# lashhw/rtcuda

Hardware: NVIDIA B200
Metric: Mrays/s (extend+shadow) (higher is better)
Workload: dtype f32

## Files before the change

rtcuda_b200/csrc/rtb_cuda.cu:

```cuda
#include <cuda_runtime.h>
#include <dlfcn.h>
#include <nccl.h>

#include <cctype>
#include <cstdlib>
#include <mutex>

#include <cub/block/block_scan.cuh>
#include <cub/device/device_radix_sort.cuh>
#include <cub/device/device_scan.cuh>
#include <cub/device/device_select.cuh>

#include "rtb_engine.h"

#define RTB_CUDA_CHECK(expr)                                                                              \
    do {                                                                                                  \
        cudaError_t e_ = (expr);                                                                          \
        if (e_ != cudaSuccess)                                                                            \
            throw rtb::Error(e_ == cudaErrorMemoryAllocation ? RTB_ERR_OOM : RTB_ERR_CUDA,                \
                             std::string(#expr) + ": " + cudaGetErrorName(e_) + " (" + cudaGetErrorString(e_) + ")"); \
    } while (0)

namespace rtb {

constexpr int kBlock = 256;
#ifndef RTB_TRACE_BLOCK
#define RTB_TRACE_BLOCK 128
#endif
constexpr int kTraceBlock = RTB_TRACE_BLOCK;
#ifndef RTB_TRACE_MIN_BLOCKS
#define RTB_TRACE_MIN_BLOCKS (1024 / RTB_TRACE_BLOCK)
#endif
constexpr int kTraceBlocksPerSm = RTB_TRACE_MIN_BLOCKS;

template <class F>
__global__ void __launch_bounds__(kBlock) k_for(int n, F f) {
    const int i = blockIdx.x * kBlock + threadIdx.x;
    if (i < n) f(i);
}

__global__ void __launch_bounds__(kBlock) k_generate(WaveState W, RenderConsts rc) {
    const int n = generate_count(W);
    for (int i = blockIdx.x * kBlock + threadIdx.x; i < n; i += gridDim.x * kBlock) generate_body(W, rc, i);
}

__device__ __forceinline__ void prefetch_l2(const void *p) { asm volatile("prefetch.global.L2 [%0];" ::"l"(p)); }

__device__ __forceinline__ void cp_async16(void *smem, const void *gmem) {
    asm volatile("cp.async.cg.shared.global [%0], [%1], 16;" ::"r"((unsigned)__cvta_generic_to_shared(smem)), "l"(gmem));
}
#ifndef RTB_SHADE_BLOCK
#define RTB_SHADE_BLOCK 128
#endif
constexpr int kShadeBlock = RTB_SHADE_BLOCK;
#ifndef RTB_SHADE_MATTE_BLOCKS
#define RTB_SHADE_MATTE_BLOCKS 2
#endif
constexpr int shade_blocks_per_sm(int type) { return ((type == RTB_MIRROR || type == RTB_GLASS) ? 3 : RTB_SHADE_MATTE_BLOCKS) * (256 / kShadeBlock); }
template <int TYPE, bool EXT = false>
__global__ void __launch_bounds__(kShadeBlock, shade_blocks_per_sm(TYPE)) k_shade(WaveState W, SceneView S, RenderConsts rc, bool shadows) {
    __shared__ float4 stage[2][3][kShadeBlock];
    const int n = W.c->n_mat[TYPE];
    const int stride = gridDim.x * kShadeBlock, t = threadIdx.x;
    ShadeTally tally; tally.extend = 0u; tally.shadow = 0u;
    int i = blockIdx.x * kShadeBlock + t;
    if (i < n) {
        const size_t q = (size_t)W.qbase[TYPE] + (size_t)i;
        cp_async16(&stage[0][0][t], W.ma + q); cp_async16(&stage[0][1][t], W.mb + q); cp_async16(&stage[0][2][t], W.mc + q);
    }
    asm volatile("cp.async.commit_group;");
    for (int buf = 0; i < n; i += stride, buf ^= 1) {
        if (i + stride < n) {
            const size_t q = (size_t)W.qbase[TYPE] + (size_t)(i + stride);
            cp_async16(&stage[buf ^ 1][0][t], W.ma + q); cp_async16(&stage[buf ^ 1][1][t], W.mb + q); cp_async16(&stage[buf ^ 1][2][t], W.mc + q);
        }
        asm volatile("cp.async.commit_group;");
        asm volatile("cp.async.wait_group 1;" ::: "memory");
        const float4 a4 = stage[buf][0][t], b4 = stage[buf][1][t], h4 = stage[buf][2][t];
        F4 a, b, hr;
        a.x = a4.x; a.y = a4.y; a.z = a4.z; a.w = a4.w; b.x = b4.x; b.y = b4.y; b.z = b4.z; b.w = b4.w;
        hr.x = h4.x; hr.y = h4.y; hr.z = h4.z; hr.w = h4.w;
        shade_item<TYPE, EXT>(W, S, rc, shadows, i, a, b, hr, tally);
    }
    asm volatile("cp.async.wait_all;" ::: "memory");
    tally_flush(W.c, tally);
}

__global__ void k_control(WaveState W, bool shadows) { control_body(W, shadows); }

struct FetchTuning {
    int refill;
    int chunk;
    int prefetch;
    int tri_step;
};

struct alignas(16) WarpScratch {
    float4 ro[32];
    float4 rd[32];
    float4 fin[32];
    float4 res[32];
    uint2 item[32];
};
template <bool ANY>
__device__ __forceinline__ void pooled_triangles(WarpScratch &ws, const Bvh8View &B, Traversal<ANY, false> &T, uint32_t tx,
                                                 uint32_t ty, bool &has, bool &pending, const unsigned lane,
                                                 const unsigned lanes_below) {
    while (__any_sync(0xffffffffu, ty != 0u)) {
        const int cnt = min(__popc(ty), 3);
        const unsigned b0 = __ballot_sync(0xffffffffu, cnt & 1), b1 = __ballot_sync(0xffffffffu, cnt & 2);
        const int first = __popc(b0 & lanes_below) + 2 * __popc(b1 & lanes_below);
        const int total = __popc(b0) + 2 * __popc(b1);
        const int take = max(0, min(cnt, 32 - first));
#pragma unroll
        for (int k = 0; k < 3; ++k) {
            if (k < take) {
                const int bit = 31 - __clz(ty);
                ty &= ~(1u << bit);
                ws.item[first + k] = make_uint2(tx + (uint32_t)bit, lane);
            }
        }
        __syncwarp();
        if ((int)lane < min(total, 32)) {
            const uint2 it = ws.item[lane];
            const float4 o = ws.ro[it.y], d = ws.rd[it.y];
            const Tri48 tr = load_tri(B.tris, (int)it.x);
            float u, v;
            const float t = tri_candidate(tr, v3(o.x, o.y, o.z), v3(d.x, d.y, d.z), u, v);
            ws.res[lane] = make_float4(t, u, v, __int_as_float((int)it.x));
        }
        __syncwarp();
#pragma unroll
        for (int k = 0; k < 3; ++k) {
            if (k < take && has) {
                const float4 c = ws.res[first + k];
                if (T.accept(B, __float_as_int(c.w), c.x, c.y, c.z)) {
                    ty = 0u; has = false; pending = true;
                }
            }
        }
        __syncwarp();
    }
}
template <bool ANY>
__device__ __forceinline__ void own_triangles(const Bvh8View &B, Traversal<ANY, false> &T, uint32_t tx, uint32_t ty, bool &has,
                                              bool &pending) {
    while (ty) {
        const int bit = 31 - __clz(ty);
        ty &= ~(1u << bit);
        const int idx = (int)(tx + (uint32_t)bit);
        const Tri48 tr = load_tri(B.tris, idx);
        float u, v;
        const float t = tri_candidate(tr, T.r.o, T.r.d, u, v);
        if (T.accept(B, idx, t, u, v)) { has = false; pending = true; break; }
    }
}

struct LocalStackK : LocalStack {
    __device__ explicit LocalStackK(uint2 *) {}
};
template <int N>
struct HybridStack {
    uint2 *s;
    uint32_t x[kStackSize - N], y[kStackSize - N];
    __device__ explicit HybridStack(uint2 *column) : s(column) {}
    __device__ __forceinline__ void put(int i, uint32_t a, uint32_t b) {
        if (i < N) s[i * kTraceBlock] = make_uint2(a, b);
        else { x[i - N] = a; y[i - N] = b; }
    }
    __device__ __forceinline__ void get(int i, uint32_t &a, uint32_t &b) const {
        if (i < N) { const uint2 v = s[i * kTraceBlock]; a = v.x; b = v.y; }
        else { a = x[i - N]; b = y[i - N]; }
    }
};
template <bool ANY, bool POOL, bool INST = false, class STACK = LocalStackK>
__device__ __forceinline__ void persistent_trace(WarpScratch &ws, const WaveState &W, const SceneView &S, FetchTuning tune, uint2 *ws_stack = nullptr) {
    const int n = ANY ? W.c->n_shadow : W.c->n_extend;
    int32_t *head = ANY ? &W.c->shadow_head : &W.c->extend_head;
    const unsigned lane = threadIdx.x & 31u;
    const unsigned lanes_below = (1u << lane) - 1u;
    Traversal<ANY, false, INST> T;
    STACK st(ws_stack);
    bool has = false, exhausted = false, pending = false;
    int qi = 0;
    int chunk_next = 0, chunk_end = 0;
    uint32_t tx = 0u, ty = 0u;
    while (true) {
        if (pending) {
            asm volatile("cp.async.wait_all;" ::: "memory");
            const float4 fw = ws.fin[lane];
            if (ANY) {
                if (!T.found) {
                    const V3 L = v3(fw.x, fw.y, fw.z);
                    if (finite3(L)) accum_add(W, __float_as_uint(fw.w), L);
                }
            } else if (T.hit.tri < 0) {
                if (W.has_env) extend_miss(W, __float_as_uint(ws.ro[lane].w), v3(fw.x, fw.y, fw.z));
            } else {
                const int mat = INST ? hit_material(S, T.hit.tri, T.hit_inst) : S.tri_meta[T.hit.tri].material;
                const int type = mat >> 24;
                const int j = hit_queue_push(W, type);
                if (INST) W.hit_inst[j] = T.hit_inst;
                F4 beta; beta.x = fw.x; beta.y = fw.y; beta.z = fw.z; beta.w = fw.w;
                const float4 o = ws.ro[lane], d = ws.rd[lane];
                F4 ma; ma.x = d.x; ma.y = d.y; ma.z = d.z; ma.w = o.w;
                F4 mb; mb.x = beta.x; mb.y = beta.y; mb.z = beta.z; mb.w = d.w;
                F4 mc; mc.x = i2f(mat); mc.y = T.hit.u; mc.z = T.hit.v; mc.w = i2f(T.hit.tri);
                W.ma[j] = ma; W.mb[j] = mb; W.mc[j] = mc;
                if (W.mis) { W.mis[2 * (size_t)j] = beta.w; W.mis[2 * (size_t)j + 1] = T.hit.t; }
            }
            pending = false;
        }
        unsigned need = __ballot_sync(0xffffffffu, !has);
        for (int round = 0; round < 2 && need != 0u && !exhausted; ++round) {
            if (chunk_next >= chunk_end) {
                int base = 0;
                if (lane == 0u) base = atomicAdd(head, tune.chunk);
                base = __shfl_sync(0xffffffffu, base, 0);
                chunk_next = base;
                chunk_end = min(base + tune.chunk, n);
                if (base >= n) { exhausted = true; break; }
                if (tune.prefetch) {
                    for (int i = base + (int)lane; i < chunk_end; i += 32) {
                        if (ANY) { prefetch_l2(W.sh_o + i); prefetch_l2(W.sh_d + i); }
                        else { prefetch_l2(W.ea + i); prefetch_l2(W.eb + i); prefetch_l2(W.ec + i); }
                    }
                }
            }
            const int idx = chunk_next + __popc(need & lanes_below);
            if (!has && idx < chunk_end) {
                if (ANY) {
                    const F4 o = ldg(W.sh_o + idx), d = ldg(W.sh_d + idx);
                    if (o.w > 0.f) {
                        cp_async16(&ws.fin[lane], W.sh_L + idx);
                        ws.ro[lane] = make_float4(o.x, o.y, o.z, 0.f);
                        ws.rd[lane] = make_float4(d.x, d.y, d.z, 0.f);
                        T.init(xyz(o), xyz(d), o.w, f2i(d.w));
                        qi = idx; has = true; ty = 0u;
                    }
                } else {
                    const F4 a = ldg(W.ea + idx), b = ldg(W.eb + idx);
                    if (f2u(a.w) != kHolePixel) {
                        cp_async16(&ws.fin[lane], W.ec + idx);
                        ws.ro[lane] = make_float4(a.x, a.y, a.z, a.w);
                        ws.rd[lane] = make_float4(b.x, b.y, b.z, b.w);
                        T.init(xyz(a), xyz(b), FLT_MAX, -1);
                        qi = idx; has = true; ty = 0u;
                    }
                }
            }
            chunk_next = min(chunk_next + __popc(need), chunk_end);
            need = __ballot_sync(0xffffffffu, !has);
        }
        unsigned act = __ballot_sync(0xffffffffu, has);
        if (act == 0u) {
            if (exhausted) return;
            continue;
        }
        const int keep_going = exhausted ? 1 : tune.refill;
        do {
            if constexpr (INST) {
                if (has && ty == 0u) T.node_part(S.bvh, st, tx, ty);
                if (has && T.cur < 0) {
                    if (ty != 0u) {
                        const float4 o = ws.ro[lane], d = ws.rd[lane];
                        T.enter_instance(S.bvh, st, tx, ty, v3(o.x, o.y, o.z), v3(d.x, d.y, d.z));
                    }
                } else if (ty != 0u) {
// ... 11 lines not shown
                    else if (two && T.accept(S.bvh, idx2, t2, u2, v2)) { has = false; pending = true; ty = 0u; }
                }
                if (has && ty == 0u) {
                    const float4 o = ws.ro[lane], d = ws.rd[lane];
                    if (!T.advance_inst(st, tx, ty, v3(o.x, o.y, o.z), v3(d.x, d.y, d.z))) { has = false; pending = true; }
                }
            } else if constexpr (POOL) {
                tx = 0u; ty = 0u;
                if (has) T.node_part(S.bvh, st, tx, ty);
                pooled_triangles<ANY>(ws, S.bvh, T, tx, ty, has, pending, lane, lanes_below);
                ty = 0u;
                if (has && !T.advance(st)) { has = false; pending = true; }
            } else if (tune.tri_step > 0) {
                if (has && ty == 0u) T.node_part(S.bvh, st, tx, ty);
                if (tune.tri_step == 2) {
                  if (ty != 0u) {
                    const int bit1 = 31 - __clz(ty);
                    ty &= ~(1u << bit1);
                    const bool two = ty != 0u;
                    const int bit2 = two ? 31 - __clz(ty) : bit1;
                    ty &= ~(1u << bit2);
                    const int idx1 = (int)(tx + (uint32_t)bit1), idx2 = (int)(tx + (uint32_t)bit2);
                    const Tri48 tr1 = load_tri(S.bvh.tris, idx1), tr2 = load_tri(S.bvh.tris, idx2);
                    float u1, v1, u2, v2;
                    const float t1 = tri_candidate(tr1, T.r.o, T.r.d, u1, v1);
                    const float t2 = tri_candidate(tr2, T.r.o, T.r.d, u2, v2);
                    if (T.accept(S.bvh, idx1, t1, u1, v1)) { has = false; pending = true; ty = 0u; }
                    else if (two && T.accept(S.bvh, idx2, t2, u2, v2)) { has = false; pending = true; ty = 0u; }
                  }
                } else {
#pragma unroll 1
                for (int k = 0; k < tune.tri_step && ty != 0u; ++k) {
                    const int bit = 31 - __clz(ty);
                    ty &= ~(1u << bit);
                    const int idx = (int)(tx + (uint32_t)bit);
                    const Tri48 tr = load_tri(S.bvh.tris, idx);
                    float u, v;
                    const float t = tri_candidate(tr, T.r.o, T.r.d, u, v);
                    if (T.accept(S.bvh, idx, t, u, v)) { has = false; pending = true; ty = 0u; }
                }
                }
                if (has && ty == 0u && !T.advance(st)) { has = false; pending = true; }
            } else {
                tx = 0u; ty = 0u;
                if (has) T.node_part(S.bvh, st, tx, ty);
                own_triangles<ANY>(S.bvh, T, tx, ty, has, pending);
                ty = 0u;
                if (has && !T.advance(st)) { has = false; pending = true; }
            }
            act = __ballot_sync(0xffffffffu, has);
        } while (__popc(act) >= keep_going);
    }
}
template <int WHICH, bool POOL, bool INST = false>
__global__ void __launch_bounds__(kTraceBlock, kTraceBlocksPerSm) k_trace(WaveState W, SceneView S, FetchTuning tune) {
    __shared__ WarpScratch scratch[kTraceBlock / 32];
    WarpScratch &ws = scratch[threadIdx.x >> 5];
    if (WHICH & 1) persistent_trace<false, POOL, INST>(ws, W, S, tune);
    if (WHICH == 3) __syncwarp();
    if (WHICH & 2) persistent_trace<true, POOL, INST>(ws, W, S, tune);
}
constexpr int kSmemStack = 8;
__global__ void __launch_bounds__(kTraceBlock, kTraceBlocksPerSm) k_trace_smem_stack(WaveState W, SceneView S, FetchTuning tune) {
    __shared__ WarpScratch scratch[kTraceBlock / 32];
    __shared__ uint2 sstack[kSmemStack][kTraceBlock];
    WarpScratch &ws = scratch[threadIdx.x >> 5];
    persistent_trace<false, false, false, HybridStack<kSmemStack>>(ws, W, S, tune, &sstack[0][threadIdx.x]);
    __syncwarp();
    persistent_trace<true, false, false, HybridStack<kSmemStack>>(ws, W, S, tune, &sstack[0][threadIdx.x]);
}
template <int WHICH>
static void launch_trace_kernel(int grid, cudaStream_t st, bool pooled, bool smem_stack, const WaveState &W, const SceneView &S, const FetchTuning &tune) {
    if (WHICH == 3 && smem_stack && !S.bvh.inst && !pooled) { k_trace_smem_stack<<<grid, kTraceBlock, 0, st>>>(W, S, tune); return; }
    if (S.bvh.inst) {
        k_trace<WHICH, false, true><<<grid, kTraceBlock, 0, st>>>(W, S, tune);
    } else if (pooled) k_trace<WHICH, true><<<grid, kTraceBlock, 0, st>>>(W, S, tune);
    else k_trace<WHICH, false><<<grid, kTraceBlock, 0, st>>>(W, S, tune);
}
template <bool COUNT>
__global__ void __launch_bounds__(kBlock) k_extend_flat(WaveState W, SceneView S) {
    const int i = blockIdx.x * kBlock + threadIdx.x;
    if (i < W.c->n_extend) extend_body<COUNT>(W, S, i);
}
template <bool COUNT>
__global__ void __launch_bounds__(kBlock) k_shadow_flat(WaveState W, SceneView S) {
    const int i = blockIdx.x * kBlock + threadIdx.x;
    if (i < W.c->n_shadow) shadow_body<COUNT>(W, S, i);
}

constexpr int kSetupBlock = 256;
__global__ void __launch_bounds__(kSetupBlock) k_prim_setup_tiled(PrimSetupArgs a) {
    __shared__ __align__(16) float vin[kSetupBlock * 9];
    __shared__ float4 rec[kSetupBlock * 3];
    const int b0 = blockIdx.x * kSetupBlock;
    const int cnt = min(kSetupBlock, a.n - b0);
    const float *src = a.vertices + 9 * (size_t)b0;
    if (cnt == kSetupBlock && (reinterpret_cast<uintptr_t>(src) & 15u) == 0) {
        const float4 *s4 = reinterpret_cast<const float4 *>(src);
        float4 *d4 = reinterpret_cast<float4 *>(vin);
        for (int t = threadIdx.x; t < kSetupBlock * 9 / 4; t += kSetupBlock) d4[t] = s4[t];
    } else {
        for (int t = threadIdx.x; t < cnt * 9; t += kSetupBlock) vin[t] = src[t];
    }
    __syncthreads();
    const int i = b0 + threadIdx.x;
    Tri48 tr;
    if (i < a.n) {
        const float *v = vin + 9 * threadIdx.x;
        tr = tri_from_vertices(v3(v[0], v[1], v[2]), v3(v[3], v[4], v[5]), v3(v[6], v[7], v[8]));
        float4 *r = rec + 3 * threadIdx.x;
        r[0] = make_float4(tr.p0x, tr.p0y, tr.p0z, tr.e1x);
        r[1] = make_float4(tr.e1y, tr.e1z, tr.e2x, tr.e2y);
        r[2] = make_float4(tr.e2z, tr.nx, tr.ny, tr.nz);
    }
    __syncthreads();
    float4 *dst = reinterpret_cast<float4 *>(a.tri_in + b0);
    for (int t = threadIdx.x; t < cnt * 3; t += kSetupBlock) dst[t] = rec[t];
    __shared__ int32_t part[kSetupBlock / 32][6];
    int32_t o[6] = {0x7fffffff, 0x7fffffff, 0x7fffffff, (int32_t)0x80000000, (int32_t)0x80000000, (int32_t)0x80000000};
    if (i < a.n) {
        V3 lo, hi;
        prim_setup_box(a, i, tr, lo, hi);
        o[0] = float_to_ordered(lo.x); o[1] = float_to_ordered(lo.y); o[2] = float_to_ordered(lo.z);
        o[3] = float_to_ordered(hi.x); o[4] = float_to_ordered(hi.y); o[5] = float_to_ordered(hi.z);
    }
#pragma unroll
    for (int k = 0; k < 3; ++k) { o[k] = __reduce_min_sync(0xffffffffu, o[k]); o[3 + k] = __reduce_max_sync(0xffffffffu, o[3 + k]); }
    if ((threadIdx.x & 31) == 0) for (int k = 0; k < 6; ++k) part[threadIdx.x >> 5][k] = o[k];
    __syncthreads();
    if (threadIdx.x < 6) {
// ... 350 lines not shown
    decltype(&ncclGetUniqueId) GetUniqueId = nullptr;
    decltype(&ncclCommInitRank) CommInitRank = nullptr;
    decltype(&ncclCommInitAll) CommInitAll = nullptr;
    decltype(&ncclCommDestroy) CommDestroy = nullptr;
    decltype(&ncclAllReduce) AllReduce = nullptr;
    decltype(&ncclReduce) Reduce = nullptr;
    decltype(&ncclGroupStart) GroupStart = nullptr;
    decltype(&ncclGroupEnd) GroupEnd = nullptr;
    decltype(&ncclGetErrorString) GetErrorString = nullptr;
    static Nccl &get() {
        static Nccl n;
        static std::once_flag once;
        std::call_once(once, [] {
            for (const char *name : {"libnccl.so.2", "libnccl.so"}) {
                n.lib = dlopen(name, RTLD_NOW | RTLD_GLOBAL);
                if (n.lib) break;
            }
            if (!n.lib) return;
#define RTB_NCCL_SYM(f) n.f = (decltype(n.f))dlsym(n.lib, "nccl" #f)
            RTB_NCCL_SYM(GetUniqueId); RTB_NCCL_SYM(CommInitRank); RTB_NCCL_SYM(CommInitAll); RTB_NCCL_SYM(CommDestroy);
            RTB_NCCL_SYM(AllReduce); RTB_NCCL_SYM(Reduce); RTB_NCCL_SYM(GroupStart); RTB_NCCL_SYM(GroupEnd); RTB_NCCL_SYM(GetErrorString);
#undef RTB_NCCL_SYM
        });
        if (!n.lib || !n.GetUniqueId || !n.CommInitRank || !n.CommInitAll || !n.CommDestroy || !n.AllReduce || !n.Reduce || !n.GroupStart ||
            !n.GroupEnd || !n.GetErrorString)
            throw Error(RTB_ERR_NO_DEVICE, "NCCL (libnccl.so.2) could not be loaded: multi-GPU entry points need it");
        return n;
    }
};
#define RTB_NCCL_CHECK(expr)                                                                                               \
    do {                                                                                                                   \
        ncclResult_t r_ = (expr);                                                                                          \
        if (r_ != ncclSuccess) throw rtb::Error(RTB_ERR_CUDA, std::string(#expr) + ": " + rtb::Nccl::get().GetErrorString(r_)); \
    } while (0)
static_assert(sizeof(ncclUniqueId) == RTB_COMM_ID_BYTES, "rtb.h: RTB_COMM_ID_BYTES must be sizeof(ncclUniqueId)");

struct NonNegative {
    __host__ __device__ bool operator()(const int32_t &v) const { return v >= 0; }
};

struct CudaBackend {
    int dev_ = -1;
    int num_sms_ = 0;
    cudaStream_t stream_ = nullptr;
    cudaStream_t streams_[kMaxPipelines] = {nullptr, nullptr};
    cudaEvent_t sync_ev_ = nullptr;
    cudaMemPool_t pool_mem_ = nullptr;
    int pipelines_ = 0;
    int blocks_trace_ = 0, blocks_generate_ = 0;
    int trace_blocks_per_sm_ = 1, trace_cap_ = 0, active_pipelines_ = 1;
    void *cub_temp_ = nullptr;
    size_t cub_temp_bytes_ = 0;
    int32_t *h_done_ = nullptr, *d_done_ = nullptr;
    FetchTuning tune_{24, 128, 1, 2};
    int pooled_ = 0;
    int fused_ = 1;
    int smem_stack_ = 0;
    WaveCache wave_cache_;
    WaveCache &wave_cache() { return wave_cache_; }
    int pool_ = 0;
    size_t pool_budget_ = 0;
    int ploc_tail_off_ = 0;
    int nn_tiled_off_ = 0;

    explicit CudaBackend(int device) {
        int count = 0;
        cudaError_t e = cudaGetDeviceCount(&count);
        if (e != cudaSuccess || count == 0)
            throw Error(RTB_ERR_NO_DEVICE, std::string("no CUDA device available (") + cudaGetErrorString(e) +
                                               "); rtcuda_b200 has no CPU fallback");
        if (device < 0 || device >= count) throw Error(RTB_ERR_INVALID, "device ordinal out of range");
        cudaDeviceProp prop;
        RTB_CUDA_CHECK(cudaGetDeviceProperties(&prop, device));
        if (prop.major != 10)
            throw Error(RTB_ERR_NO_DEVICE, std::string("device '") + prop.name + "' is sm_" + std::to_string(prop.major) +
                                               std::to_string(prop.minor) + "; this library is built for sm_100a (B200) only");
        dev_ = device;
        num_sms_ = prop.multiProcessorCount;
        RTB_CUDA_CHECK(cudaSetDevice(dev_));
        for (int k = 0; k < kMaxPipelines; ++k) RTB_CUDA_CHECK(cudaStreamCreateWithFlags(&streams_[k], cudaStreamDefault));
        stream_ = streams_[0];
        RTB_CUDA_CHECK(cudaEventCreateWithFlags(&sync_ev_, cudaEventDisableTiming));
        cudaMemPoolProps props = {};
        props.allocType = cudaMemAllocationTypePinned;
        props.handleTypes = cudaMemHandleTypeNone;
        props.location.type = cudaMemLocationTypeDevice;
        props.location.id = dev_;
        RTB_CUDA_CHECK(cudaMemPoolCreate(&pool_mem_, &props));
        unsigned long long keep = ~0ull;
        RTB_CUDA_CHECK(cudaMemPoolSetAttribute(pool_mem_, cudaMemPoolAttrReleaseThreshold, &keep));
        {
            size_t free_b = 0, total_b = 0;
            RTB_CUDA_CHECK(cudaMemGetInfo(&free_b, &total_b));
            pool_budget_ = free_b / 8;
        }
        RTB_CUDA_CHECK(cudaHostAlloc((void **)&h_done_, kMaxPipelines * sizeof(int32_t), cudaHostAllocMapped));
        RTB_CUDA_CHECK(cudaHostGetDevicePointer((void **)&d_done_, h_done_, 0));
        for (int k = 0; k < kMaxPipelines; ++k) h_done_[k] = 0;
        int per_sm = 0;
        RTB_CUDA_CHECK(cudaOccupancyMaxActiveBlocksPerMultiprocessor(&per_sm, k_trace<3, true>, kTraceBlock, 0));
        trace_blocks_per_sm_ = per_sm > 0 ? per_sm : 1;
        static const char *const names[] = {"refill", "chunk", "prefetch", "tri_step", "pooled", "fused", "smem_stack", "pipelines", "pool",
                                            "ploc_tail", "trace_blocks", "nn_tiled"};
        for (const char *nm : names) {
            std::string env = "RTB_";
            for (const char *c = nm; *c; ++c) env += (char)toupper((unsigned char)*c);
            if (const char *e = getenv(env.c_str())) set_option(nm, atoll(e));
        }
        blocks_trace_ = num_sms_ * trace_blocks_per_sm_;
        RTB_CUDA_CHECK(cudaOccupancyMaxActiveBlocksPerMultiprocessor(&per_sm, k_generate, kBlock, 0));
        blocks_generate_ = num_sms_ * (per_sm > 0 ? per_sm : 1);
    }
    ~CudaBackend() {
        if (dev_ < 0) return;
        cudaSetDevice(dev_);
        stream_ = streams_[0];
        for (int k = 0; k < kMaxPipelines; ++k) if (streams_[k]) cudaStreamSynchronize(streams_[k]);
        wave_cache_release(*this, wave_cache_);
        if (cub_temp_) cudaFreeAsync(cub_temp_, stream_);
        if (tail_counts_) cudaFreeAsync(tail_counts_, stream_);
        if (h_done_) cudaFreeHost(h_done_);
        if (sync_ev_) cudaEventDestroy(sync_ev_);
        for (int k = 0; k < kMaxPipelines; ++k) if (streams_[k]) { cudaStreamSynchronize(streams_[k]); cudaStreamDestroy(streams_[k]); }
        if (pool_mem_) cudaMemPoolDestroy(pool_mem_);
    }
    CudaBackend(const CudaBackend &) = delete;
    CudaBackend &operator=(const CudaBackend &) = delete;

    bool set_option(const std::string &name, long long v) {
        auto in = [&](long long lo, long long hi) { return v >= lo && v <= hi; };
        if (name == "refill") { if (!in(1, 32)) return false; tune_.refill = (int)v; }
        else if (name == "chunk") { if (!in(32, 1 << 20)) return false; tune_.chunk = (int)v; }
        else if (name == "prefetch") { if (!in(0, 1)) return false; tune_.prefetch = (int)v; }
        else if (name == "tri_step") { if (!in(0, 4)) return false; tune_.tri_step = (int)v; }
        else if (name == "pooled") { if (!in(-1, 1)) return false; pooled_ = (int)v; }
        else if (name == "fused") { if (!in(0, 1)) return false; fused_ = (int)v; }
        else if (name == "smem_stack") { if (!in(0, 1)) return false; smem_stack_ = (int)v; }
        else if (name == "pipelines") { if (!in(0, kMaxPipelines)) return false; pipelines_ = (int)v; }
        else if (name == "pool") { if (v != 0 && !in(1024, 1ll << 30)) return false; pool_ = (int)v; }
        else if (name == "ploc_tail") { if (!in(0, 1)) return false; ploc_tail_off_ = v == 0; }
        else if (name == "trace_blocks") { if (!in(0, trace_blocks_per_sm_)) return false; trace_cap_ = (int)v; }
        else if (name == "nn_tiled") { if (!in(0, 1)) return false; nn_tiled_off_ = v == 0; }
        else return false;
        return true;
    }
    bool get_option(const std::string &name, long long &v) const {
        if (name == "refill") v = tune_.refill;
        else if (name == "chunk") v = tune_.chunk;
        else if (name == "prefetch") v = tune_.prefetch;
        else if (name == "tri_step") v = tune_.tri_step;
        else if (name == "pooled") v = pooled_;
        else if (name == "fused") v = fused_;
        else if (name == "smem_stack") v = smem_stack_;
        else if (name == "pipelines") v = pipelines_;
        else if (name == "pool") v = pool_;
        else if (name == "ploc_tail") v = ploc_tail_off_ ? 0 : 1;
        else if (name == "trace_blocks") v = trace_cap_;
        else if (name == "nn_tiled") v = nn_tiled_off_ ? 0 : 1;
        else return false;
        return true;
    }
    int device() const { return dev_; }
    void make_current() { RTB_CUDA_CHECK(cudaSetDevice(dev_)); }
    void sync() { RTB_CUDA_CHECK(cudaStreamSynchronize(stream_)); }
    long long default_pool(size_t slot_bytes) const {
        if (pool_ > 0) return pool_;
        long long n = (long long)(pool_budget_ / (slot_bytes ? slot_bytes : 144));
        if (n < (1ll << 22)) n = 1ll << 22;
        if (n > (1ll << 28)) n = 1ll << 28;
        return n;
    }

    template <class T> T *alloc(size_t n) {
        void *p = nullptr;
        RTB_CUDA_CHECK(cudaMallocFromPoolAsync(&p, sizeof(T) * (n ? n : 1), pool_mem_, stream_));
        return (T *)p;
    }
    void free(void *p) { if (p) cudaFreeAsync(p, stream_); }
    template <class T> void upload(T *dst, const T *src, size_t n) {
        RTB_CUDA_CHECK(cudaMemcpyAsync(dst, src, sizeof(T) * n, cudaMemcpyHostToDevice, stream_));
        RTB_CUDA_CHECK(cudaStreamSynchronize(stream_));
    }
    template <class T> void download(T *dst, const T *src, size_t n) {
        RTB_CUDA_CHECK(cudaMemcpyAsync(dst, src, sizeof(T) * n, cudaMemcpyDeviceToHost, stream_));
        RTB_CUDA_CHECK(cudaStreamSynchronize(stream_));
    }
    template <class T> void copy(T *dst, const T *src, size_t n) {
        RTB_CUDA_CHECK(cudaMemcpyAsync(dst, src, sizeof(T) * n, cudaMemcpyDeviceToDevice, stream_));
    }
    template <class T> void zero(T *p, size_t n) { RTB_CUDA_CHECK(cudaMemsetAsync(p, 0, sizeof(T) * n, stream_)); }
    template <class T> void copy_from(CudaBackend &src_be, T *dst, const T *src, size_t n) {
        if (!n) return;
        if (src_be.dev_ == dev_) { copy(dst, src, n); return; }
        RTB_CUDA_CHECK(cudaMemcpyPeerAsync(dst, dev_, src, src_be.dev_, sizeof(T) * n, stream_));
    }
    struct Group { std::vector<ncclComm_t> comms; };
    static Group *group_create(const std::vector<CudaBackend *> &members) {
        Nccl &nc = Nccl::get();
        std::vector<int> devs;
        for (CudaBackend *b : members) devs.push_back(b->dev_);
        Group *g = new Group();
        g->comms.resize(members.size());
        ncclResult_t r = nc.CommInitAll(g->comms.data(), (int)devs.size(), devs.data());
        if (r != ncclSuccess) { delete g; throw Error(RTB_ERR_CUDA, std::string("ncclCommInitAll: ") + nc.GetErrorString(r)); }
        return g;
    }
    static void group_destroy(Group *g) {
        if (!g) return;
        for (ncclComm_t c : g->comms) if (c) Nccl::get().CommDestroy(c);
        delete g;
    }
    template <class T>
    static void group_reduce(Group *g, const std::vector<CudaBackend *> &members, const std::vector<T *> &bufs, size_t n, int root) {
        Nccl &nc = Nccl::get();
        const ncclDataType_t dt = sizeof(T) == 8 ? ncclInt64 : ncclFloat32;
        RTB_NCCL_CHECK(nc.GroupStart());
        for (size_t r = 0; r < members.size(); ++r) {
            ncclResult_t e = nc.Reduce(bufs[r], bufs[r], n, dt, ncclSum, root, g->comms[r], members[r]->streams_[0]);
            if (e != ncclSuccess) { nc.GroupEnd(); throw Error(RTB_ERR_CUDA, std::string("ncclReduce: ") + nc.GetErrorString(e)); }
        }
        RTB_NCCL_CHECK(nc.GroupEnd());
    }
    struct Comm { ncclComm_t comm = nullptr; int rank = 0, world = 1; };
    static void comm_unique_id(uint8_t *out) {
        ncclUniqueId id;
        RTB_NCCL_CHECK(Nccl::get().GetUniqueId(&id));
        memcpy(out, &id, sizeof id);
    }
    Comm *comm_create(const uint8_t *id_bytes, int rank, int world) {
        ncclUniqueId id;
        memcpy(&id, id_bytes, sizeof id);
        make_current();
        Comm *c = new Comm();
        c->rank = rank; c->world = world;
        ncclResult_t r = Nccl::get().CommInitRank(&c->comm, world, id, rank);
        if (r != ncclSuccess) { delete c; throw Error(RTB_ERR_CUDA, std::string("ncclCommInitRank: ") + Nccl::get().GetErrorString(r)); }
        return c;
    }
    static void comm_destroy(Comm *c) {
        if (!c) return;
        if (c->comm) Nccl::get().CommDestroy(c->comm);
        delete c;
    }
    template <class T> void comm_allreduce(Comm *c, T *buf, size_t n) {
        const ncclDataType_t dt = sizeof(T) == 8 ? ncclInt64 : ncclFloat32;
        RTB_NCCL_CHECK(Nccl::get().AllReduce(buf, buf, n, dt, ncclSum, c->comm, streams_[0]));
        RTB_CUDA_CHECK(cudaStreamSynchronize(streams_[0]));
    }

    template <class F> void launch(int n, F f) {
        if (n <= 0) return;
        k_for<F><<<(n + kBlock - 1) / kBlock, kBlock, 0, stream_>>>(n, f);
        RTB_CUDA_CHECK(cudaGetLastError());
    }
    template <class F> void launch_trace(int n, F f) { launch(n, f); }
    void generate(const GenerateK &k) {
        k_generate<<<blocks_generate_, kBlock, 0, stream_>>>(k.W, k.rc);
        RTB_CUDA_CHECK(cudaGetLastError());
    }
    void shade(const ShadeK &k) {
        const int grid = num_sms_ * shade_blocks_per_sm(k.type);
        if ((k.rc.flags & (RTB_RENDER_TRUE_MIS | RTB_RENDER_RR_TERMINATE)) || k.S.bvh.inst) {
            if (k.type == 0) k_shade<0, true><<<grid, kShadeBlock, 0, stream_>>>(k.W, k.S, k.rc, k.shadows);
            else if (k.type == 1) k_shade<1, true><<<grid, kShadeBlock, 0, stream_>>>(k.W, k.S, k.rc, k.shadows);
            else if (k.type == 2) k_shade<2, true><<<grid, kShadeBlock, 0, stream_>>>(k.W, k.S, k.rc, k.shadows);
            else k_shade<3, true><<<grid, kShadeBlock, 0, stream_>>>(k.W, k.S, k.rc, k.shadows);
        } else {
            if (k.type == 0) k_shade<0><<<grid, kShadeBlock, 0, stream_>>>(k.W, k.S, k.rc, k.shadows);
            else if (k.type == 1) k_shade<1><<<grid, kShadeBlock, 0, stream_>>>(k.W, k.S, k.rc, k.shadows);
            else if (k.type == 2) k_shade<2><<<grid, kShadeBlock, 0, stream_>>>(k.W, k.S, k.rc, k.shadows);
            else k_shade<3><<<grid, kShadeBlock, 0, stream_>>>(k.W, k.S, k.rc, k.shadows);
        }
        RTB_CUDA_CHECK(cudaGetLastError());
    }
    void control(const WaveState &W, bool shadows) {
        k_control<<<1, 1, 0, stream_>>>(W, shadows);
        RTB_CUDA_CHECK(cudaGetLastError());
    }
    void begin_render(int pipelines) { active_pipelines_ = pipelines; }
    int trace_grid(const SceneView &S) const {
        int per = trace_blocks_per_sm_;
        if (trace_cap_ > 0) per = trace_cap_;
        else if (active_pipelines_ > 1 && !big_scene(S)) per = per / active_pipelines_ > 0 ? per / active_pipelines_ : 1;
        return num_sms_ * per;
    }
    bool big_scene(const SceneView &S) const {
        return (size_t)S.bvh.num_nodes * 80 + (size_t)S.bvh.num_tris * 48 > ((size_t)48 << 20);
    }
    bool use_pooled(const SceneView &S) const { return pooled_ < 0 ? big_scene(S) : pooled_ != 0; }
    void extend(const WaveState &W, const SceneView &S, int mode) {
        const int flat_grid = (W.pool + kBlock - 1) / kBlock;
        if (mode == 2) k_extend_flat<true><<<flat_grid, kBlock, 0, stream_>>>(W, S);
        else if (mode == 1) k_extend_flat<false><<<flat_grid, kBlock, 0, stream_>>>(W, S);
        else launch_trace_kernel<1>(trace_grid(S), stream_, use_pooled(S), smem_stack_ != 0, W, S, tune_);
        RTB_CUDA_CHECK(cudaGetLastError());
    }
    void shadow(const WaveState &W, const SceneView &S, int mode) {
        const int flat_grid = (W.pool + kBlock - 1) / kBlock;
        if (mode == 2) k_shadow_flat<true><<<flat_grid, kBlock, 0, stream_>>>(W, S);
        else if (mode == 1) k_shadow_flat<false><<<flat_grid, kBlock, 0, stream_>>>(W, S);
        else launch_trace_kernel<2>(trace_grid(S), stream_, use_pooled(S), smem_stack_ != 0, W, S, tune_);
        RTB_CUDA_CHECK(cudaGetLastError());
    }
    bool trace_fused(const WaveState &W, const SceneView &S, int mode) {
        if (mode != 0 || !fused_) return false;
        launch_trace_kernel<3>(trace_grid(S), stream_, use_pooled(S), smem_stack_ != 0, W, S, tune_);
        RTB_CUDA_CHECK(cudaGetLastError());
        return true;
    }
    int pipelines(const SceneView &S) const { return pipelines_ > 0 ? pipelines_ : (big_scene(S) ? 2 : 4); }
    void use_stream(int k) { stream_ = streams_[k]; }
    void fork(int k) {
        RTB_CUDA_CHECK(cudaEventRecord(sync_ev_, streams_[0]));
        RTB_CUDA_CHECK(cudaStreamWaitEvent(streams_[k], sync_ev_, 0));
    }
    void join(int k) {
        RTB_CUDA_CHECK(cudaEventRecord(sync_ev_, streams_[k]));
        RTB_CUDA_CHECK(cudaStreamWaitEvent(streams_[0], sync_ev_, 0));
    }
    int32_t *done_flag_device(int k) { return d_done_ + k; }
    void reset_done(int k) { ((volatile int32_t *)h_done_)[k] = 0; }
    bool done(int k) const { return ((volatile int32_t *)h_done_)[k] != 0; }
    void wait(cudaEvent_t e) { RTB_CUDA_CHECK(cudaEventSynchronize(e)); }

    void ensure_temp(size_t bytes) {
        if (bytes <= cub_temp_bytes_) return;
        if (cub_temp_) cudaFreeAsync(cub_temp_, stream_);
        cub_temp_ = nullptr; cub_temp_bytes_ = 0;
        RTB_CUDA_CHECK(cudaMallocFromPoolAsync(&cub_temp_, bytes, pool_mem_, stream_));
        cub_temp_bytes_ = bytes;
    }
    void sort_pairs(uint64_t *keys, int32_t *vals, int n) {
        uint64_t *k2 = alloc<uint64_t>(n);
        int32_t *v2 = alloc<int32_t>(n);
        cub::DoubleBuffer<uint64_t> dk(keys, k2);
        cub::DoubleBuffer<int32_t> dv(vals, v2);
        size_t bytes = 0;
        RTB_CUDA_CHECK(cub::DeviceRadixSort::SortPairs(nullptr, bytes, dk, dv, n, 0, 63, stream_));
        ensure_temp(bytes);
        RTB_CUDA_CHECK(cub::DeviceRadixSort::SortPairs(cub_temp_, bytes, dk, dv, n, 0, 63, stream_));
        if (dk.Current() != keys) copy(keys, dk.Current(), n);
        if (dv.Current() != vals) copy(vals, dv.Current(), n);
        free(k2); free(v2);
    }
    void prim_setup(const PrimSetupArgs &a) {
        if (a.n <= 0) return;
        if (!a.vertices) { PrimSetupK k; k.a = a; launch(a.n, k); return; }
        k_prim_setup_tiled<<<(a.n + kSetupBlock - 1) / kSetupBlock, kSetupBlock, 0, stream_>>>(a);
        RTB_CUDA_CHECK(cudaGetLastError());
    }
    void ploc_nn(const PlocArgs &a) {
        if (a.ncl <= 0) return;
        if (a.radius > kNnMaxRadius || nn_tiled_off_) { PlocNnK k; k.a = a; launch(a.ncl, k); return; }
        k_ploc_nn_tiled<<<(a.ncl + kNnBlock - 1) / kNnBlock, kNnBlock, 0, stream_>>>(a);
        RTB_CUDA_CHECK(cudaGetLastError());
    }
    int32_t *tail_counts_ = nullptr;
    int32_t *ploc_tail_counts() {
        if (!tail_counts_) tail_counts_ = alloc<int32_t>(kPlocTail);
        return tail_counts_;
// ... 84 lines not shown
```

rtcuda_b200/csrc/rtb_engine.h:

```cpp
#pragma once
#include <algorithm>
#include <cmath>
#include <stdexcept>
#include <string>
#include <type_traits>
#include <vector>

#include "rtb_build.h"
#include "rtb_wavefront.h"

namespace rtb {

struct Error : std::runtime_error {
    int code;
    Error(int c, const std::string &m) : std::runtime_error(m), code(c) {}
};

template <class BE, class T>
struct DeviceBuf {
    BE &be; T *p;
    DeviceBuf(BE &b, size_t n) : be(b), p(n ? b.template alloc<T>(n) : nullptr) {}
    ~DeviceBuf() { be.free(p); }
    DeviceBuf(const DeviceBuf &) = delete;
    DeviceBuf &operator=(const DeviceBuf &) = delete;
// ... 1418 lines not shown
                       rtb_render_stats *stats) {
    if (p.width <= 0 || p.height <= 0 || p.spp <= 0 || p.max_bounces < 0 || !(target.add_f32 || target.add_fixed || target.tonemap_to))
        throw Error(RTB_ERR_INVALID, "rtb_render: bad parameters");
    if (p.device_mask != 0 && be.device() >= 0 && !(p.device_mask >> be.device() & 1))
        throw Error(RTB_ERR_INVALID, "rtb_render: device_mask excludes the GPU of this scene's context (use rtb_multi_render to span GPUs)");
    if (p.max_bounces > kMaxBounces) throw Error(RTB_ERR_INVALID, "rtb_render: max_bounces > 255");
    if (p.first_sample < 0 || (long long)p.first_sample + p.spp > kMaxSampleIndex) throw Error(RTB_ERR_INVALID, "rtb_render: sample index >= 2^24");
    const unsigned long long total = (unsigned long long)p.width * (unsigned long long)p.height * (unsigned long long)p.spp;
    if ((unsigned long long)p.width * (unsigned long long)p.height > 0x7fffffffull) throw Error(RTB_ERR_INVALID, "image too large");
    const int mode = (p.flags & RTB_RENDER_COUNT_WORK) ? 2 : ((p.flags & RTB_RENDER_NONPERSISTENT) ? 1 : 0);
    const size_t slot_bytes = 96 + (size_t)sc.num_present() * (48 + ((p.flags & RTB_RENDER_TRUE_MIS) ? 8 : 0) + (sc.inst ? 4 : 0));
    long long pool_all = p.pool_size > 0 ? p.pool_size : be.default_pool(slot_bytes);
    if ((unsigned long long)pool_all > total) pool_all = (long long)total;
    int np = be.pipelines(sc.view());
    if (np > kMaxPipelines) np = kMaxPipelines;
    if (np < 1 || mode != 0 || (p.flags & RTB_RENDER_SINGLE_PIPELINE) || pool_all < (1 << 16)) np = 1;
    const int pool = (int)(((pool_all + np - 1) / np + 31) & ~31ll);
    sc.ensure_wave(pool, np);
    const bool fixed = (p.flags & RTB_RENDER_DETERMINISTIC) != 0 || target.add_fixed != nullptr;
    const int64_t pixels = (int64_t)p.width * p.height;
    if (3 * pixels > 0x7fffff00ll) throw Error(RTB_ERR_INVALID, "image too large");
    sc.ensure_accum(pixels, fixed);
    const SceneView S = sc.view();
    const bool shadows = sc.num_lights > 0 && !(p.flags & RTB_RENDER_NO_SHADOW);
    WaveState W[kMaxPipelines];
    RenderConsts rc[kMaxPipelines];
    be.use_stream(0);
    be.begin_render(np);
    auto t0 = be.now();
    if (fixed) be.zero(sc.accum_fx, 3 * (size_t)pixels);
    else be.zero(sc.accum, (size_t)pixels);
    for (int k = 0; k < np; ++k) {
        if ((p.flags & RTB_RENDER_TRUE_MIS) && !sc.W[k].mis) sc.W[k].mis = be.template alloc<float>(2 * (size_t)sc.num_present() * (size_t)pool);
        W[k] = sc.W[k];
        if (!(p.flags & RTB_RENDER_TRUE_MIS)) W[k].mis = nullptr;
        W[k].env[0] = p.env_L[0]; W[k].env[1] = p.env_L[1]; W[k].env[2] = p.env_L[2];
        W[k].has_env = (p.env_L[0] != 0.f || p.env_L[1] != 0.f || p.env_L[2] != 0.f) ? 1 : 0;
        W[k].accum = fixed ? nullptr : sc.accum;
        W[k].accum_fx = fixed ? sc.accum_fx : nullptr;
        W[k].host_done = be.done_flag_device(k);
        RenderConsts &r = rc[k];
        r.cam = cam; r.width = p.width; r.height = p.height; r.spp = p.spp; r.first_sample = p.first_sample;
        r.max_bounces = p.max_bounces; r.rr_start = p.rr_start; r.rr_threshold = p.rr_threshold; r.seed = p.seed; r.flags = p.flags;
        r.path_offset = k; r.path_stride = np;
        r.env[0] = p.env_L[0]; r.env[1] = p.env_L[1]; r.env[2] = p.env_L[2];
        Counters c0;
        memset(&c0, 0, sizeof c0);
        c0.total_paths = (total - (unsigned long long)k + (unsigned long long)np - 1ull) / (unsigned long long)np;
        be.reset_done(k);
        be.upload(W[k].c, &c0, 1);
    }
    for (int k = 1; k < np; ++k) be.fork(k);
    unsigned long long launches = 0;
    const int batch = 4;
    const bool time_stages = stats != nullptr && np == 1;
    std::vector<typename BE::Time> stage_times, fences[kMaxPipelines];
    size_t fence_head[kMaxPipelines] = {0, 0};
    bool finished[kMaxPipelines] = {false, false};
    bool fused = false;
    int live = np;
    while (live > 0) {
        for (int k = 0; k < np; ++k) {
            if (finished[k]) continue;
            be.use_stream(k);
            for (int b = 0; b < batch; ++b) {
                if (time_stages) stage_times.push_back(be.now());
                for (int type = 0; type < kNumMaterialTypes; ++type) {
                    if (!(sc.type_mask >> type & 1u)) continue;
                    ShadeK ks; ks.W = W[k]; ks.S = S; ks.rc = rc[k]; ks.type = type; ks.shadows = shadows;
                    be.shade(ks);
                    ++launches;
                }
                { GenerateK kg; kg.W = W[k]; kg.rc = rc[k]; be.generate(kg); }
                be.control(W[k], shadows);
                if (time_stages) stage_times.push_back(be.now());
                if (be.trace_fused(W[k], S, mode)) {
                    fused = true;
                    if (time_stages) { stage_times.push_back(be.now()); stage_times.push_back(be.now()); }
                    launches += 3;
                } else {
                    be.extend(W[k], S, mode);
                    if (time_stages) stage_times.push_back(be.now());
                    be.shadow(W[k], S, mode);
                    if (time_stages) stage_times.push_back(be.now());
                    launches += 4;
                }
            }
            fences[k].push_back(be.now());
        }
        for (int k = 0; k < np; ++k) {
            if (finished[k]) continue;
            if (fences[k].size() - fence_head[k] > 2) be.wait(fences[k][fence_head[k]++]);
            if (be.done(k)) { finished[k] = true; --live; }
        }
    }
    be.use_stream(0);
    for (int k = 1; k < np; ++k) be.join(k);
    if (target.add_f32) {
        FoldF32K k; k.in = sc.accum; k.in_fx = fixed ? sc.accum_fx : nullptr; k.out = target.add_f32; k.pixels = pixels;
        be.launch((int)pixels, k);
    }
    if (target.add_fixed) { FoldFixedK k; k.in_fx = sc.accum_fx; k.out = target.add_fixed; k.n = 3 * pixels; be.launch((int)(3 * pixels), k); }
    if (target.tonemap_to) {
        if (target.tonemap_spp <= 0) throw Error(RTB_ERR_INVALID, "rtb_render: bad total_spp");
        TonemapAccumK k; k.in = sc.accum; k.in_fx = fixed ? sc.accum_fx : nullptr; k.out = target.tonemap_to; k.pixels = pixels;
        k.inv_spp = 1.0f / (float)target.tonemap_spp;
        be.launch((int)pixels, k);
    }
    auto t1 = be.now();
    be.wait(t1);
    for (int k = 0; k < np; ++k) for (auto &e : fences[k]) be.release(e);
    float ms_extend = 0.f, ms_shadow = 0.f, ms_shade = 0.f;
    for (size_t i = 0; i + 3 < stage_times.size(); i += 4) {
        ms_shade += be.elapsed_keep(stage_times[i], stage_times[i + 1]);
        ms_extend += be.elapsed_keep(stage_times[i + 1], stage_times[i + 2]);
        ms_shadow += be.elapsed_keep(stage_times[i + 2], stage_times[i + 3]);
    }
    for (auto &e : stage_times) be.release(e);
    const float ms_total = be.elapsed_ms(t0, t1);
    if (stats) {
        memset(stats, 0, sizeof *stats);
        for (int k = 0; k < np; ++k) {
            Counters c;
            be.download(&c, W[k].c, 1);
            stats->paths += c.stat_paths;
            stats->extend_rays += c.stat_extend;
            stats->shadow_rays += c.stat_shadow;
            stats->iterations += c.stat_iters;
            stats->extend_nodes += c.work[0]; stats->extend_tris += c.work[1];
            stats->shadow_nodes += c.work[2]; stats->shadow_tris += c.work[3];
            stats->hits += c.stat_hits;
        }
        stats->kernel_launches = launches;
        stats->extend_launches = stats->iterations; stats->shadow_launches = stats->iterations;
        stats->ms_extend = ms_extend; stats->ms_shadow = ms_shadow;
        stats->ms_total = ms_total;
        stats->ms_other = ms_total - ms_extend - ms_shadow;
        stats->ms_shade = ms_shade;
        stats->fused_trace = fused ? 1 : 0;
        stats->pipelines = np;
        stats->pool = pool;
    }
}

struct RayLoadK {
// ... 127 lines not shown
```

Before: 18110.

## Add trace claim budget, stage launch priorities, and shrink host launch batching

Adds an optional per-block claim budget to the persistent trace kernels, with extra short-lived blocks and an early exit when the queues are already drained. Adds optional high-priority launches for the generate/shade/control stages and creates all streams at the lowest priority. Independently, the host loop now issues 2 waves per batch instead of 4 and waits once more than 1 fence is outstanding instead of 2, which tightens host-device coupling. The budget and priority features are off by default. The batching change and the move to cudaLaunchKernelEx are always active, so the net effect mostly comes from less queued work ahead of the host.

```diff
diff --git a/rtcuda_b200/csrc/rtb_cuda.cu b/rtcuda_b200/csrc/rtb_cuda.cu
--- a/rtcuda_b200/csrc/rtb_cuda.cu
+++ b/rtcuda_b200/csrc/rtb_cuda.cu
@@ -3,6 +3,7 @@
 #include <nccl.h>
 
 #include <cctype>
+#include <climits>
 #include <cstdlib>
 #include <mutex>
 
@@ -93,6 +94,8 @@
     int chunk;
     int prefetch;
     int tri_step;
+    int budget;
+    int budget_blocks;
 };
 
 struct alignas(16) WarpScratch {
@@ -173,8 +176,9 @@
         else { a = x[i - N]; b = y[i - N]; }
     }
 };
-template <bool ANY, bool POOL, bool INST = false, class STACK = LocalStackK>
-__device__ __forceinline__ void persistent_trace(WarpScratch &ws, const WaveState &W, const SceneView &S, FetchTuning tune, uint2 *ws_stack = nullptr) {
+template <bool ANY, bool POOL, bool INST = false, class STACK = LocalStackK, bool BUDGET = false>
+__device__ __forceinline__ void persistent_trace(WarpScratch &ws, const WaveState &W, const SceneView &S, FetchTuning tune, int &claims_left,
+                                                 uint2 *ws_stack = nullptr) {
     const int n = ANY ? W.c->n_shadow : W.c->n_extend;
     int32_t *head = ANY ? &W.c->shadow_head : &W.c->extend_head;
     const unsigned lane = threadIdx.x & 31u;
@@ -214,6 +218,10 @@
         unsigned need = __ballot_sync(0xffffffffu, !has);
         for (int round = 0; round < 2 && need != 0u && !exhausted; ++round) {
             if (chunk_next >= chunk_end) {
+                if (BUDGET) {
+                    if (claims_left == 0) { exhausted = true; break; }
+                    --claims_left;
+                }
                 int base = 0;
                 if (lane == 0u) base = atomicAdd(head, tune.chunk);
                 base = __shfl_sync(0xffffffffu, base, 0);
@@ -331,30 +339,58 @@
         } while (__popc(act) >= keep_going);
     }
 }
-template <int WHICH, bool POOL, bool INST = false>
+template <int WHICH, bool BUDGET>
+__device__ __forceinline__ int trace_claims(const WaveState &W, const FetchTuning &tune) {
+    if (!BUDGET) return 0;
+    bool drained = true;
+    if (WHICH & 1) drained = *(volatile const int32_t *)&W.c->extend_head >= W.c->n_extend;
+    if (WHICH & 2) drained = drained && *(volatile const int32_t *)&W.c->shadow_head >= W.c->n_shadow;
+    if (__all_sync(0xffffffffu, drained)) return -1;
+    return (int)blockIdx.x < tune.budget_blocks ? tune.budget : INT_MAX;
+}
+template <int WHICH, bool POOL, bool INST = false, bool BUDGET = false>
 __global__ void __launch_bounds__(kTraceBlock, kTraceBlocksPerSm) k_trace(WaveState W, SceneView S, FetchTuning tune) {
     __shared__ WarpScratch scratch[kTraceBlock / 32];
     WarpScratch &ws = scratch[threadIdx.x >> 5];
-    if (WHICH & 1) persistent_trace<false, POOL, INST>(ws, W, S, tune);
+    int claims = trace_claims<WHICH, BUDGET>(W, tune);
+    if (BUDGET && claims < 0) return;
+    if (WHICH & 1) persistent_trace<false, POOL, INST, LocalStackK, BUDGET>(ws, W, S, tune, claims);
     if (WHICH == 3) __syncwarp();
-    if (WHICH & 2) persistent_trace<true, POOL, INST>(ws, W, S, tune);
+    if (WHICH & 2) persistent_trace<true, POOL, INST, LocalStackK, BUDGET>(ws, W, S, tune, claims);
 }
 constexpr int kSmemStack = 8;
+template <bool BUDGET>
 __global__ void __launch_bounds__(kTraceBlock, kTraceBlocksPerSm) k_trace_smem_stack(WaveState W, SceneView S, FetchTuning tune) {
     __shared__ WarpScratch scratch[kTraceBlock / 32];
     __shared__ uint2 sstack[kSmemStack][kTraceBlock];
     WarpScratch &ws = scratch[threadIdx.x >> 5];
-    persistent_trace<false, false, false, HybridStack<kSmemStack>>(ws, W, S, tune, &sstack[0][threadIdx.x]);
+    int claims = trace_claims<3, BUDGET>(W, tune);
+    if (BUDGET && claims < 0) return;
+    persistent_trace<false, false, false, HybridStack<kSmemStack>, BUDGET>(ws, W, S, tune, claims, &sstack[0][threadIdx.x]);
     __syncwarp();
-    persistent_trace<true, false, false, HybridStack<kSmemStack>>(ws, W, S, tune, &sstack[0][threadIdx.x]);
-}
-template <int WHICH>
-static void launch_trace_kernel(int grid, cudaStream_t st, bool pooled, bool smem_stack, const WaveState &W, const SceneView &S, const FetchTuning &tune) {
-    if (WHICH == 3 && smem_stack && !S.bvh.inst && !pooled) { k_trace_smem_stack<<<grid, kTraceBlock, 0, st>>>(W, S, tune); return; }
+    persistent_trace<true, false, false, HybridStack<kSmemStack>, BUDGET>(ws, W, S, tune, claims, &sstack[0][threadIdx.x]);
+}
+template <class... P, class... A>
+static void launch_at(void (*kernel)(P...), int grid, int block, cudaStream_t st, bool raise, int prio, A &&...args) {
+    cudaLaunchConfig_t cfg = {};
+    cfg.gridDim = dim3((unsigned)grid);
+    cfg.blockDim = dim3((unsigned)block);
+    cfg.stream = st;
+    cudaLaunchAttribute attr[1];
+    attr[0].id = cudaLaunchAttributePriority;
+    attr[0].val.priority = prio;
+    cfg.attrs = attr;
+    cfg.numAttrs = raise ? 1 : 0;
+    RTB_CUDA_CHECK(cudaLaunchKernelEx(&cfg, kernel, std::forward<A>(args)...));
+}
+template <int WHICH, bool BUDGET>
+static void launch_trace_kernel(int grid, cudaStream_t st, bool pooled, bool smem_stack, const WaveState &W, const SceneView &S,
+                                const FetchTuning &tune) {
+    if (WHICH == 3 && smem_stack && !S.bvh.inst && !pooled) { launch_at(k_trace_smem_stack<BUDGET>, grid, kTraceBlock, st, false, 0, W, S, tune); return; }
     if (S.bvh.inst) {
-        k_trace<WHICH, false, true><<<grid, kTraceBlock, 0, st>>>(W, S, tune);
-    } else if (pooled) k_trace<WHICH, true><<<grid, kTraceBlock, 0, st>>>(W, S, tune);
-    else k_trace<WHICH, false><<<grid, kTraceBlock, 0, st>>>(W, S, tune);
+        launch_at(k_trace<WHICH, false, true, BUDGET>, grid, kTraceBlock, st, false, 0, W, S, tune);
+    } else if (pooled) launch_at(k_trace<WHICH, true, false, BUDGET>, grid, kTraceBlock, st, false, 0, W, S, tune);
+    else launch_at(k_trace<WHICH, false, false, BUDGET>, grid, kTraceBlock, st, false, 0, W, S, tune);
 }
 template <bool COUNT>
 __global__ void __launch_bounds__(kBlock) k_extend_flat(WaveState W, SceneView S) {
@@ -811,7 +847,10 @@
     void *cub_temp_ = nullptr;
     size_t cub_temp_bytes_ = 0;
     int32_t *h_done_ = nullptr, *d_done_ = nullptr;
-    FetchTuning tune_{24, 128, 1, 2};
+    FetchTuning tune_{24, 128, 1, 2, 0, 0};
+    int trace_budget_ = 0;
+    int stage_priority_ = 0;
+    int prio_least_ = 0, prio_greatest_ = 0;
     int pooled_ = 0;
     int fused_ = 1;
     int smem_stack_ = 0;
@@ -837,7 +876,8 @@
         dev_ = device;
         num_sms_ = prop.multiProcessorCount;
         RTB_CUDA_CHECK(cudaSetDevice(dev_));
-        for (int k = 0; k < kMaxPipelines; ++k) RTB_CUDA_CHECK(cudaStreamCreateWithFlags(&streams_[k], cudaStreamDefault));
+        RTB_CUDA_CHECK(cudaDeviceGetStreamPriorityRange(&prio_least_, &prio_greatest_));
+        for (int k = 0; k < kMaxPipelines; ++k) RTB_CUDA_CHECK(cudaStreamCreateWithPriority(&streams_[k], cudaStreamDefault, prio_least_));
         stream_ = streams_[0];
         RTB_CUDA_CHECK(cudaEventCreateWithFlags(&sync_ev_, cudaEventDisableTiming));
         cudaMemPoolProps props = {};
@@ -900,6 +940,8 @@
         else if (name == "ploc_tail") { if (!in(0, 1)) return false; ploc_tail_off_ = v == 0; }
         else if (name == "trace_blocks") { if (!in(0, trace_blocks_per_sm_)) return false; trace_cap_ = (int)v; }
         else if (name == "nn_tiled") { if (!in(0, 1)) return false; nn_tiled_off_ = v == 0; }
+        else if (name == "trace_budget") { if (!in(0, 1 << 16)) return false; trace_budget_ = (int)v; }
+        else if (name == "stage_priority") { if (!in(0, 1)) return false; stage_priority_ = (int)v; }
         else return false;
         return true;
     }
@@ -916,6 +958,8 @@
         else if (name == "ploc_tail") v = ploc_tail_off_ ? 0 : 1;
         else if (name == "trace_blocks") v = trace_cap_;
         else if (name == "nn_tiled") v = nn_tiled_off_ ? 0 : 1;
+        else if (name == "trace_budget") v = trace_budget_;
+        else if (name == "stage_priority") v = stage_priority_;
         else return false;
         return true;
     }
@@ -1013,35 +1057,50 @@
         RTB_CUDA_CHECK(cudaGetLastError());
     }
     template <class F> void launch_trace(int n, F f) { launch(n, f); }
-    void generate(const GenerateK &k) {
-        k_generate<<<blocks_generate_, kBlock, 0, stream_>>>(k.W, k.rc);
-        RTB_CUDA_CHECK(cudaGetLastError());
-    }
+    template <class... P, class... A>
+    void launch_stage(bool raise, void (*kernel)(P...), int grid, int block, A &&...args) {
+        launch_at(kernel, grid, block, stream_, raise, prio_greatest_, std::forward<A>(args)...);
+    }
+    void generate(const GenerateK &k) { launch_stage(stage_priority_ != 0, k_generate, blocks_generate_, kBlock, k.W, k.rc); }
     void shade(const ShadeK &k) {
         const int grid = num_sms_ * shade_blocks_per_sm(k.type);
         if ((k.rc.flags & (RTB_RENDER_TRUE_MIS | RTB_RENDER_RR_TERMINATE)) || k.S.bvh.inst) {
-            if (k.type == 0) k_shade<0, true><<<grid, kShadeBlock, 0, stream_>>>(k.W, k.S, k.rc, k.shadows);
-            else if (k.type == 1) k_shade<1, true><<<grid, kShadeBlock, 0, stream_>>>(k.W, k.S, k.rc, k.shadows);
-            else if (k.type == 2) k_shade<2, true><<<grid, kShadeBlock, 0, stream_>>>(k.W, k.S, k.rc, k.shadows);
-            else k_shade<3, true><<<grid, kShadeBlock, 0, stream_>>>(k.W, k.S, k.rc, k.shadows);
+            if (k.type == 0) launch_stage(stage_priority_ != 0, k_shade<0, true>, grid, kShadeBlock, k.W, k.S, k.rc, k.shadows);
+            else if (k.type == 1) launch_stage(stage_priority_ != 0, k_shade<1, true>, grid, kShadeBlock, k.W, k.S, k.rc, k.shadows);
+            else if (k.type == 2) launch_stage(stage_priority_ != 0, k_shade<2, true>, grid, kShadeBlock, k.W, k.S, k.rc, k.shadows);
+            else launch_stage(stage_priority_ != 0, k_shade<3, true>, grid, kShadeBlock, k.W, k.S, k.rc, k.shadows);
         } else {
-            if (k.type == 0) k_shade<0><<<grid, kShadeBlock, 0, stream_>>>(k.W, k.S, k.rc, k.shadows);
-            else if (k.type == 1) k_shade<1><<<grid, kShadeBlock, 0, stream_>>>(k.W, k.S, k.rc, k.shadows);
-            else if (k.type == 2) k_shade<2><<<grid, kShadeBlock, 0, stream_>>>(k.W, k.S, k.rc, k.shadows);
-            else k_shade<3><<<grid, kShadeBlock, 0, stream_>>>(k.W, k.S, k.rc, k.shadows);
-        }
-        RTB_CUDA_CHECK(cudaGetLastError());
-    }
-    void control(const WaveState &W, bool shadows) {
-        k_control<<<1, 1, 0, stream_>>>(W, shadows);
-        RTB_CUDA_CHECK(cudaGetLastError());
-    }
+            if (k.type == 0) launch_stage(stage_priority_ != 0, k_shade<0>, grid, kShadeBlock, k.W, k.S, k.rc, k.shadows);
+            else if (k.type == 1) launch_stage(stage_priority_ != 0, k_shade<1>, grid, kShadeBlock, k.W, k.S, k.rc, k.shadows);
+            else if (k.type == 2) launch_stage(stage_priority_ != 0, k_shade<2>, grid, kShadeBlock, k.W, k.S, k.rc, k.shadows);
+            else launch_stage(stage_priority_ != 0, k_shade<3>, grid, kShadeBlock, k.W, k.S, k.rc, k.shadows);
+        }
+    }
+    void control(const WaveState &W, bool shadows) { launch_stage(stage_priority_ != 0, k_control, 1, 1, W, shadows); }
     void begin_render(int pipelines) { active_pipelines_ = pipelines; }
-    int trace_grid(const SceneView &S) const {
+    int resident_trace_grid(const SceneView &S) const {
         int per = trace_blocks_per_sm_;
         if (trace_cap_ > 0) per = trace_cap_;
         else if (active_pipelines_ > 1 && !big_scene(S)) per = per / active_pipelines_ > 0 ? per / active_pipelines_ : 1;
         return num_sms_ * per;
+    }
+    int trace_grid(const WaveState &W, const SceneView &S, FetchTuning &tune) const {
+        const int resident = resident_trace_grid(S);
+        tune.budget = trace_budget_;
+        if (tune.budget == 0) { tune.budget_blocks = 0; return resident; }
+        const long long per_block = (long long)tune.budget * tune.chunk * (kTraceBlock / 32);
+        long long limited = (2ll * W.pool + per_block - 1) / per_block;
+        if (limited > INT_MAX - resident) limited = INT_MAX - resident;
+        tune.budget_blocks = (int)limited;
+        return tune.budget_blocks + resident;
+    }
+    template <int WHICH>
+    void persistent_launch(const WaveState &W, const SceneView &S) {
+        FetchTuning tune = tune_;
+        const int grid = trace_grid(W, S, tune);
+        if (tune.budget > 0) launch_trace_kernel<WHICH, true>(grid, stream_, use_pooled(S), smem_stack_ != 0, W, S, tune);
+        else launch_trace_kernel<WHICH, false>(grid, stream_, use_pooled(S), smem_stack_ != 0, W, S, tune);
+        RTB_CUDA_CHECK(cudaGetLastError());
     }
     bool big_scene(const SceneView &S) const {
         return (size_t)S.bvh.num_nodes * 80 + (size_t)S.bvh.num_tris * 48 > ((size_t)48 << 20);
@@ -1051,20 +1110,19 @@
         const int flat_grid = (W.pool + kBlock - 1) / kBlock;
         if (mode == 2) k_extend_flat<true><<<flat_grid, kBlock, 0, stream_>>>(W, S);
         else if (mode == 1) k_extend_flat<false><<<flat_grid, kBlock, 0, stream_>>>(W, S);
-        else launch_trace_kernel<1>(trace_grid(S), stream_, use_pooled(S), smem_stack_ != 0, W, S, tune_);
+        else { persistent_launch<1>(W, S); return; }
         RTB_CUDA_CHECK(cudaGetLastError());
     }
     void shadow(const WaveState &W, const SceneView &S, int mode) {
         const int flat_grid = (W.pool + kBlock - 1) / kBlock;
         if (mode == 2) k_shadow_flat<true><<<flat_grid, kBlock, 0, stream_>>>(W, S);
         else if (mode == 1) k_shadow_flat<false><<<flat_grid, kBlock, 0, stream_>>>(W, S);
-        else launch_trace_kernel<2>(trace_grid(S), stream_, use_pooled(S), smem_stack_ != 0, W, S, tune_);
+        else { persistent_launch<2>(W, S); return; }
         RTB_CUDA_CHECK(cudaGetLastError());
     }
     bool trace_fused(const WaveState &W, const SceneView &S, int mode) {
         if (mode != 0 || !fused_) return false;
-        launch_trace_kernel<3>(trace_grid(S), stream_, use_pooled(S), smem_stack_ != 0, W, S, tune_);
-        RTB_CUDA_CHECK(cudaGetLastError());
+        persistent_launch<3>(W, S);
         return true;
     }
     int pipelines(const SceneView &S) const { return pipelines_ > 0 ? pipelines_ : (big_scene(S) ? 2 : 4); }
diff --git a/rtcuda_b200/csrc/rtb_engine.h b/rtcuda_b200/csrc/rtb_engine.h
--- a/rtcuda_b200/csrc/rtb_engine.h
+++ b/rtcuda_b200/csrc/rtb_engine.h
@@ -1494,7 +1494,7 @@
     }
     for (int k = 1; k < np; ++k) be.fork(k);
     unsigned long long launches = 0;
-    const int batch = 4;
+    const int batch = 2;
     const bool time_stages = stats != nullptr && np == 1;
     std::vector<typename BE::Time> stage_times, fences[kMaxPipelines];
     size_t fence_head[kMaxPipelines] = {0, 0};
@@ -1532,7 +1532,7 @@
         }
         for (int k = 0; k < np; ++k) {
             if (finished[k]) continue;
-            if (fences[k].size() - fence_head[k] > 2) be.wait(fences[k][fence_head[k]++]);
+            if (fences[k].size() - fence_head[k] > 1) be.wait(fences[k][fence_head[k]++]);
             if (be.done(k)) { finished[k] = true; --live; }
         }
     }
```

Result: no change. 18200 (median of 6 runs) (+0.5%).
